# dalab/matrix-manifolds

Hardware: NVIDIA B200
Metric: spd4_pair_dist_grad_evals_per_sec (higher is better)
Workload: dtype f32

## Files before the change

matrix-manifolds_b200/csrc/gm_pairs_spd.cu:

```cuda
#include "gm_product.cuh"

#ifndef GM_N
#error "compile with -DGM_N=<matrix size>"
#endif

namespace gm {

template <class Op, typename T, int KMODE>
__global__ void __launch_bounds__(128)
spd_pair_kernel(Op op, PairSpec ps, const T* __restrict__ xa, const T* __restrict__ xb,
                const T* __restrict__ gout, T coef, T* __restrict__ ga, T* __restrict__ gb,
                T* __restrict__ out_d2, TargetSpec tg, LossCfg lc, T scale_sp, double* __restrict__ acc) {
  constexpr int E = Op::E;
  __shared__ double red[2][4];
  long long k = (long long)blockIdx.x * blockDim.x + threadIdx.x;
  bool active = k < ps.P;
  long long ra = -1, rb = -1;
  double loss_v = 0.0, gd2_v = 0.0;
  T gx[E], gy[E];
  if (active) {
    decode_pair(ps, k, ra, rb);
    T x[E], y[E];
    load_row<T, E>(xa, ra, x);
    load_row<T, E>(xb, rb, y);
    if constexpr (KMODE == K_FWD) {
      out_d2[k] = op.dist2(x, y);
    } else {
      T d2 = op.dist2_grad(x, y, gx, gy);
      T w;
      if constexpr (KMODE == K_BWD) {
        w = coef * gout[k];
      } else {
        T g = fetch_target_ps<T>(ps, tg, k, ra, rb);
        T m = scale_sp * d2;
        T dm;
        T lv = loss_term<T>(lc, g, m, dm);
        loss_v = (double)lv;
        gd2_v = (double)dm * (double)d2;
        w = dm * scale_sp;
        if (out_d2) out_d2[k] = d2;
      }
      GM_UNROLL for (int e = 0; e < E; ++e) { gx[e] *= w; gy[e] *= w; }
    }
  }
  if constexpr (KMODE != K_FWD) {
    if (ps.mode == GM_PAIRS_ELEMENTWISE) {
      if (active) {
        store_row<T, E>(ga, ra, gx);
        store_row<T, E>(gb, rb, gy);
      }
    } else {
      warp_accumulate_row<T, E>(ga, ra, gx);
      warp_accumulate_row<T, E>(gb, rb, gy);
    }
  }
  if constexpr (KMODE == K_FUSED) {
    block_accumulate(loss_v, acc, red[0]);
    block_accumulate(gd2_v, acc + 1, red[1]);
  }
}

template <int BYTES>
__device__ __forceinline__ void cp_async(void* smem, const void* gmem) {
  unsigned s = (unsigned)__cvta_generic_to_shared(smem);
  if constexpr (BYTES == 16)
    asm volatile("cp.async.cg.shared.global [%0], [%1], 16;\n" ::"r"(s), "l"(gmem) : "memory");
  else if constexpr (BYTES == 8)
    asm volatile("cp.async.ca.shared.global [%0], [%1], 8;\n" ::"r"(s), "l"(gmem) : "memory");
  else
    asm volatile("cp.async.ca.shared.global [%0], [%1], 4;\n" ::"r"(s), "l"(gmem) : "memory");
}
__device__ __forceinline__ void cp_async_commit() { asm volatile("cp.async.commit_group;\n" ::: "memory"); }
__device__ __forceinline__ void cp_async_wait_all() { asm volatile("cp.async.wait_group 0;\n" ::: "memory"); }
template <int PENDING>
__device__ __forceinline__ void cp_async_wait_group() { asm volatile("cp.async.wait_group %0;\n" ::"n"(PENDING) : "memory"); }

template <typename T, int E, int STAGES = 2>
struct RowStage {
  static constexpr int ROWB = E * (int)sizeof(T);
  static constexpr int CPB = (ROWB % 16 == 0) ? 16 : ((ROWB % 8 == 0) ? 8 : 4);
  static constexpr int NCH = ROWB / CPB;
  static constexpr int THREADS = 128;
  static constexpr int BYTES = STAGES * 2  * ROWB * THREADS;
  __device__ __forceinline__ static char* slot(char* base, int s, int r, int c, int t) {
    return base + ((((s * 2 + r) * NCH + c) * THREADS + t) * CPB);
  }
  __device__ __forceinline__ static void issue(char* base, int s, int r, int t, const T* row) {
    const char* g = reinterpret_cast<const char*>(row);
    GM_UNROLL for (int c = 0; c < NCH; ++c) cp_async<CPB>(slot(base, s, r, c, t), g + c * CPB);
  }
  __device__ __forceinline__ static void read(char* base, int s, int r, int t, T (&out)[E]) {
    GM_UNROLL for (int c = 0; c < NCH; ++c) {
      if constexpr (CPB == 16) {
        float4 v = *reinterpret_cast<const float4*>(slot(base, s, r, c, t));
        const T* tv = reinterpret_cast<const T*>(&v);
        GM_UNROLL for (int j = 0; j < 16 / (int)sizeof(T); ++j) out[c * (16 / (int)sizeof(T)) + j] = tv[j];
      } else if constexpr (CPB == 8) {
        float2 v = *reinterpret_cast<const float2*>(slot(base, s, r, c, t));
        const T* tv = reinterpret_cast<const T*>(&v);
        GM_UNROLL for (int j = 0; j < 8 / (int)sizeof(T); ++j) out[c * (8 / (int)sizeof(T)) + j] = tv[j];
      } else {
        out[c] = *reinterpret_cast<const T*>(slot(base, s, r, c, t));
      }
    }
  }
};

struct PairCursor {
  long long a, pos;
  int slot;
  __device__ __forceinline__ void init(const PairSpec& ps, long long k0) {
    if (ps.mode == GM_PAIRS_TRIU && k0 < ps.P) {
      long long b;
      triu_decode(k0 + ps.k0, ps.B, a, b);
      pos = b - a - 1;
    } else {
      a = -1; pos = 0; slot = 0;
    }
  }
  __device__ __forceinline__ void rows(const PairSpec& ps, long long k, long long& ra, long long& rb) const {
    if (ps.mode == GM_PAIRS_LIST) {
      ra = load_index(ps.idx_i, k, ps.idx64);
      rb = load_index(ps.idx_j, k, ps.idx64);
    } else if (ps.mode == GM_PAIRS_SAMPLED) {
      const unsigned char* hp;
      rb = (long long)sampled_j(ps, k, ra, hp);
    } else {
      long long b = a + 1 + pos;
      if (ps.nodes) { ra = load_index(ps.nodes, a, ps.idx64); rb = load_index(ps.nodes, b, ps.idx64); }
      else { ra = a; rb = b; }
    }
  }
  __device__ __forceinline__ void rows_sampled(const PairSpec& ps, long long k, long long& ra, long long& rb,
                                               unsigned& hop) {
    const int g = (int)(ps.per_shift >= 0 ? (k >> ps.per_shift) : (k / ps.per_src));
    if (g != a) {
      a = g;
      pos = ((const int*)ps.idx_i)[g];
      slot = ps.slots ? ps.slots[g] : g;
    }
    const unsigned i = (unsigned)pos;
    unsigned j = __umulhi(sample_hash32(ps.seed, (unsigned long long)k), (unsigned)(ps.n_nodes - 1));
    j += (j >= i) ? 1u : 0u;
    hop = load_hop(ps.levels + (long long)slot * ps.n_nodes + j);
    ra = (long long)i;
    rb = (long long)j;
  }
  __device__ __forceinline__ void advance(const PairSpec& ps) {
    if (ps.mode == GM_PAIRS_TRIU) {
      pos += 32;
      while (a < ps.B - 1 && pos >= ps.B - a - 1) { pos -= ps.B - a - 1; ++a; }
    }
  }
};

template <int ROWBYTES, bool SMALL = (ROWBYTES >= 64)> struct RowId { using type = long long; };
template <int ROWBYTES> struct RowId<ROWBYTES, true> { using type = unsigned; };

template <typename T> struct RawScalar;
template <> struct RawScalar<float> {
  using type = unsigned;
  __device__ __forceinline__ static unsigned pack(float v) { return __float_as_uint(v); }
  __device__ __forceinline__ static float unpack(unsigned r) { return __uint_as_float(r); }
};
template <> struct RawScalar<double> {
  using type = unsigned long long;
  __device__ __forceinline__ static unsigned long long pack(double v) { return (unsigned long long)__double_as_longlong(v); }
  __device__ __forceinline__ static double unpack(unsigned long long r) { return __longlong_as_double((long long)r); }
};

template <class Op, typename T, int KMODE, int MINB, int DEPTH, int SPEC = 0>
__global__ void __launch_bounds__(128, MINB)
spd_pair_stream_kernel(Op op, PairSpec ps, const T* __restrict__ xa, const T* __restrict__ xb,
                       const T* __restrict__ gout, T coef, T* __restrict__ ga, T* __restrict__ gb,
                       T* __restrict__ out_d2, TargetSpec tg, LossCfg lc, T scale_sp, double* __restrict__ acc,
                       long long chunk, const ShardTab sh) {
  constexpr int E = Op::E;
  constexpr int N = GM_N;
  constexpr int EU = N * (N + 1) / 2;
  constexpr int D = DEPTH;
  using Stage = RowStage<T, E, D + 1>;
  using Raw = RawScalar<T>;
  using raw_t = typename Raw::type;
  extern __shared__ __align__(16) char stage_mem[];
  __shared__ double red[2][4];
  __shared__ T hop_lut[256];
  const int tid = threadIdx.x, lane = tid & 31;
  const unsigned full = 0xffffffffu;
  const long long warp_id = (long long)blockIdx.x * 4 + (tid >> 5);
  const long long wbase = warp_id * chunk + lane;
  const int nseg = ps.nseg;
  auto locate = [&](int t, long long& k) -> bool {
    int s = 0, o = t;
    if (nseg > 1) {
      s = t / (int)chunk;
      o = t - s * (int)chunk;
      if (s >= nseg) return false;
    } else if (t >= chunk) {
      return false;
    }
    const long long in_seg = wbase + o;
    k = (long long)s * ps.seg_len + in_seg;
    return in_seg < ps.seg_len && k < ps.P;
  };
  [[maybe_unused]] auto locate_so = [&](int s, int o, long long& k) -> bool {
    if (s >= nseg) return false;
    const long long in_seg = wbase + o;
    k = (long long)s * ps.seg_len + in_seg;
    return in_seg < ps.seg_len && k < ps.P;
  };
  const bool hopsP = SPEC ? true : (KMODE == K_FUSED) && tg.mode == GM_TGT_HOPS_PACKED;
  const bool hops8 = SPEC ? true : (KMODE == K_FUSED) && (tg.mode == GM_TGT_HOPS_U8 || hopsP);
  const bool hops16 = SPEC ? false : (KMODE == K_FUSED) && tg.mode == GM_TGT_HOPS_U16;
  const bool rawj = SPEC ? true : hopsP || ps.mode == GM_PAIRS_SAMPLED;
  if (hops8) {
    for (int h = tid; h < 256; h += 128) hop_lut[h] = ((T)h * (T)h) / (T)tg.max_sq;
    __syncthreads();
  }

  using row_t = typename RowId<E * (int)sizeof(T)>::type;
  const row_t kNoRow = (row_t)-1;
  const bool sharded = SPEC ? false : sh.log2w >= 0;
  auto xrow = [&](const T* base, row_t r) -> const T* {
    if (sharded) return (const T*)sh.x[(unsigned)r & sh.mask] + (size_t)((unsigned long long)r >> sh.log2w) * E;
    return base + (size_t)r * E;
  };
  auto grow = [&](T* base, row_t r, long long& lr) -> T* {
    lr = (long long)r;
    if (sharded) { base = (T*)sh.g[(unsigned)r & sh.mask]; lr = (long long)((unsigned long long)r >> sh.log2w); }
    return base;
  };
  int tc = 0;
  PairCursor ahead;
  row_t ra[D + 2], rb[D + 2];
  raw_t tgq[D + 1];
  bool v[D + 2];
  unsigned hopn = 0;
  GM_UNROLL for (int q = 0; q < D + 2; ++q) { ra[q] = kNoRow; rb[q] = kNoRow; v[q] = false; }
  GM_UNROLL for (int q = 0; q < D + 1; ++q) tgq[q] = 0;
  const bool sampled = SPEC ? false : ps.mode == GM_PAIRS_SAMPLED;
  int stage = 0;

  auto fetch_scalar = [&](long long k, row_t ra, row_t rb) -> raw_t {
    if constexpr (KMODE == K_BWD) {
      return Raw::pack(gout[k]);
    } else {
      if (hopsP) return (raw_t)(((unsigned)rb) >> 24);
      if (hops8) return (raw_t)((const unsigned char*)tg.data)[k];
      if (hops16) return (raw_t)((const unsigned short*)tg.data)[k];
      return Raw::pack(fetch_target<T>(tg, k, (long long)ra, (long long)rb));
    }
  };
  auto scalar_value = [&](raw_t r) -> T {
    if constexpr (KMODE == K_BWD) {
      return Raw::unpack(r);
    } else {
      if (hops8) return hop_lut[r];
      if (hops16) { T h = (T)r; return (h * h) / (T)tg.max_sq; }
      return Raw::unpack(r);
    }
  };
  auto load_rows = [&](long long k, row_t& ra, row_t& rb, unsigned& hop) {
    if constexpr (SPEC != 0) {
      ra = (row_t)((const int*)ps.idx_i)[k];
      rb = (row_t)(unsigned)((const int*)ps.idx_j)[k];
      return;
    }
    long long a, b;
    if (sampled) ahead.rows_sampled(ps, k, a, b, hop);
    else ahead.rows(ps, k, a, b);
    ra = (row_t)a; rb = (row_t)b;
  };

  ahead.init(ps, wbase);
  GM_UNROLL for (int q = 0; q < D; ++q) {
    long long kq = 0;
    v[q] = locate(32 * q, kq);
    if (v[q]) {
      unsigned hop = 0;
      load_rows(kq, ra[q], rb[q], hop);
      tgq[q] = (sampled && hopsP) ? (raw_t)hop : fetch_scalar(kq, ra[q], rb[q]);
      if (rawj) rb[q] &= (row_t)0x00ffffffu;
      Stage::issue(stage_mem, q, 0, tid, xrow(xa, ra[q]));
      Stage::issue(stage_mem, q, 1, tid, xrow(xb, rb[q]));
    }
    cp_async_commit();
    ahead.advance(ps);
  }
  {
    long long kq = 0;
    v[D] = locate(32 * D, kq);
    if (v[D]) load_rows(kq, ra[D], rb[D], hopn);
  }
  [[maybe_unused]] int hs = SPEC ? (32 * (D + 1)) / (int)chunk : 0;
  [[maybe_unused]] int ho = SPEC ? 32 * (D + 1) - hs * (int)chunk : 0;

  double loss_v = 0.0, gd2_v = 0.0;
  row_t acc_row = kNoRow;
  T gacc[EU];
  GM_UNROLL for (int e = 0; e < EU; ++e) gacc[e] = (T)0;
  row_t prep_row = kNoRow;
  T ap[Op::kPrepSize];

  auto flush = [&]() {
    if (acc_row != kNoRow) {
      GM_UNROLL for (int e = 0; e < EU; ++e) gacc[e] = warp_sum(gacc[e]);
      if (lane == 0) {
        T gfull[E];
        GM_UNROLL for (int i = 0; i < N; ++i)
          GM_UNROLL for (int j = i; j < N; ++j) {
            gfull[i * N + j] = gacc[i * N - i * (i - 1) / 2 + (j - i)];
            gfull[j * N + i] = gfull[i * N + j];
          }
        long long lr;
        T* gbase = grow(ga, acc_row, lr);
        atomic_add_row<T, E>(gbase, lr, gfull);
      }
      GM_UNROLL for (int e = 0; e < EU; ++e) gacc[e] = (T)0;
      acc_row = kNoRow;
    }
  };

  const int t_end = (nseg > 1 && wbase - lane < ps.seg_len) ? nseg * (int)chunk : 0;
  while (nseg > 1 ? tc < t_end : __any_sync(full, v[0])) {
    cp_async_wait_group<D - 1>();
    const bool v0 = v[0];
    const row_t ra0 = ra[0], rb0 = rb[0];
    const raw_t tg0 = tgq[0];
    T x[E], y[E];
    if (v0) {
      Stage::read(stage_mem, stage, 1, tid, y);
      if (!Op::kCanPrep || ra0 != prep_row) Stage::read(stage_mem, stage, 0, tid, x);
    }
    tgq[D] = 0;
    if (v[D]) {
      long long kq = 0;
      if (KMODE == K_BWD || !hopsP) locate(tc + 32 * D, kq);
      tgq[D] = (sampled && hopsP) ? (raw_t)hopn : fetch_scalar(kq, ra[D], rb[D]);
      if (rawj) rb[D] &= (row_t)0x00ffffffu;
      int sn = stage + D;
      if (sn > D) sn -= D + 1;
      Stage::issue(stage_mem, sn, 0, tid, xrow(xa, ra[D]));
      Stage::issue(stage_mem, sn, 1, tid, xrow(xb, rb[D]));
    }
    cp_async_commit();
    ahead.advance(ps);
    long long kh = 0;
    if constexpr (SPEC != 0) {
      v[D + 1] = locate_so(hs, ho, kh);
      ho += 32;
      if (ho >= (int)chunk) { ho -= (int)chunk; ++hs; }
    } else {
      v[D + 1] = locate(tc + 32 * (D + 1), kh);
    }
    ra[D + 1] = kNoRow; rb[D + 1] = kNoRow;
    unsigned hop_next = 0;
    if (v[D + 1]) load_rows(kh, ra[D + 1], rb[D + 1], hop_next);

    T gx[E], gy[E];
    if (v0) {
      T d2, w;
      [[maybe_unused]] typename Op::EigState st;
      if constexpr (Op::kCanPrep) {
        if (ra0 != prep_row) { op.prep(x, ap); prep_row = ra0; }
        d2 = op.eig_forward_prepped(ap, y, st);
      } else {
        d2 = op.dist2_grad(x, y, gx, gy);
      }
      if constexpr (KMODE == K_BWD) {
        w = coef * scalar_value(tg0);
      } else {
        T m = scale_sp * d2;
        T dm;
        T lv = loss_term<T, true>(lc, scalar_value(tg0), m, dm);
        loss_v += (double)lv;
        gd2_v += (double)dm * (double)d2;
        w = dm * scale_sp;
        if (out_d2) {
          long long k0 = 0;
          locate(tc, k0);
          out_d2[k0] = d2;
        }
      }
      if constexpr (Op::kCanPrep) {
        op.eig_backward(st, w, gx, gy);
      } else {
        GM_UNROLL for (int e = 0; e < E; ++e) { gx[e] *= w; gy[e] *= w; }
      }
      long long lrb;
      T* gbb = grow(gb, rb0, lrb);
      atomic_add_row<T, E>(gbb, lrb, gy);
    }
    {
      row_t r0 = __shfl_sync(full, ra0, 0);
      bool uniform = __all_sync(full, v0 && ra0 == r0);
      if (uniform && r0 == acc_row) {
        GM_UNROLL for (int i = 0; i < N; ++i)
          GM_UNROLL for (int j = i; j < N; ++j) gacc[i * N - i * (i - 1) / 2 + (j - i)] += gx[i * N + j];
      } else {
        flush();
        if (uniform) {
          acc_row = r0;
          GM_UNROLL for (int i = 0; i < N; ++i)
            GM_UNROLL for (int j = i; j < N; ++j) gacc[i * N - i * (i - 1) / 2 + (j - i)] = gx[i * N + j];
        } else if (v0) {
          long long lra;
          T* gba = grow(ga, ra0, lra);
          atomic_add_row<T, E>(gba, lra, gx);
        }
      }
    }
    tc += 32;
    GM_UNROLL for (int q = 0; q < D + 1; ++q) { ra[q] = ra[q + 1]; rb[q] = rb[q + 1]; v[q] = v[q + 1]; }
    GM_UNROLL for (int q = 0; q < D; ++q) tgq[q] = tgq[q + 1];
    hopn = hop_next;
    stage = (stage == D) ? 0 : stage + 1;
  }
  flush();
  if constexpr (KMODE == K_FUSED) {
    block_accumulate(loss_v, acc, red[0]);
    block_accumulate(gd2_v, acc + 1, red[1]);
  }
}

template <class Op, typename T>
static int launch_op(const Op& op, const PairArgs& a) {
  if (a.ps.P <= 0) return 0;
  if (a.px) return a.sh.log2w >= 0 ? GM_EUNSUPPORTED : launch_product<SpdLead<Op>, T>(SpdLead<Op>{op}, a);
  const int threads = 128;
  long long blocks = (a.ps.P + threads - 1) / threads;
  if (blocks > 0x7fffffffLL) return GM_EINVAL;
  dim3 grid((unsigned)blocks), block(threads);
  const T* xa = (const T*)a.xa;
  const T* xb = (const T*)a.xb;
#ifndef GM_MINB_F32
#define GM_MINB_F32 4
#endif
#ifndef GM_PF_DEPTH
#define GM_PF_DEPTH 1
#endif
  constexpr int MINB = sizeof(T) == 4 ? GM_MINB_F32 : 2;
  constexpr int DEPTH = (RowStage<T, Op::E, GM_PF_DEPTH + 1>::BYTES + 3 * 1024) * MINB <= 224 * 1024 ? GM_PF_DEPTH : 1;
  using Stage = RowStage<T, Op::E, DEPTH + 1>;
  if (a.kmode != K_FWD && a.ps.mode != GM_PAIRS_ELEMENTWISE && RowStage<T, Op::E, 2>::BYTES <= 64 * 1024) {
    int dev = 0, sms = 0, occ = 0;
    cudaGetDevice(&dev);
    cudaDeviceGetAttribute(&sms, cudaDevAttrMultiProcessorCount, dev);
    auto launch_stream = [&](auto kern, auto spec_kern, const T* gout, T coef, T* out_d2, T scale, double* acc) -> int {
      cudaFuncSetAttribute(kern, cudaFuncAttributeMaxDynamicSharedMemorySize, Stage::BYTES);
      cudaOccupancyMaxActiveBlocksPerMultiprocessor(&occ, kern, threads, Stage::BYTES);
      if (occ < 1) occ = 1;
      long long max_blocks = (long long)sms * occ;
      long long want = (a.ps.P + threads - 1) / threads;
      long long nb = want < max_blocks ? want : max_blocks;
      long long warps = nb * (threads / 32);
      PairSpec ps = a.ps;
      if (ps.mode != GM_PAIRS_LIST || ps.nseg < 2 || ps.P < ps.nseg * 32LL * warps) ps.nseg = 1;
      ps.seg_len = (ps.P + ps.nseg - 1) / ps.nseg;
      long long chunk = ((ps.seg_len + warps - 1) / warps + 31) / 32 * 32;
      if (chunk * ps.nseg > 0x7fffffffLL) return GM_EINVAL;
#ifndef GM_NO_SPEC
      if constexpr (GM_N == 4 && sizeof(T) == 4 && Op::kCanPrep) {
        if (spec_kern && ps.nseg > 1 && !ps.idx64 && a.tg.mode == GM_TGT_HOPS_PACKED && a.sh.log2w < 0) {
          cudaFuncSetAttribute(spec_kern, cudaFuncAttributeMaxDynamicSharedMemorySize, Stage::BYTES);
          spec_kern<<<(unsigned)nb, threads, Stage::BYTES, a.stream>>>(op, ps, xa, xb, gout, coef, (T*)a.ga, (T*)a.gb,
                                                                    out_d2, a.tg, a.lc, scale, acc, chunk, a.sh);
          note_launch();
          return check_launch();
        }
      }
#endif
      kern<<<(unsigned)nb, threads, Stage::BYTES, a.stream>>>(op, ps, xa, xb, gout, coef, (T*)a.ga, (T*)a.gb, out_d2,
                                                             a.tg, a.lc, scale, acc, chunk, a.sh);
      note_launch();
      return check_launch();
    };
    using kern_t = decltype(&spd_pair_stream_kernel<Op, T, K_FUSED, MINB, DEPTH>);
    if (a.kmode == K_BWD)
      return launch_stream(spd_pair_stream_kernel<Op, T, K_BWD, MINB, DEPTH>, (kern_t) nullptr, (const T*)a.gout,
                           (T)a.coef, nullptr, (T)0, nullptr);
    kern_t spec = nullptr;
    if constexpr (GM_N == 4 && sizeof(T) == 4 && Op::kCanPrep) spec = spd_pair_stream_kernel<Op, T, K_FUSED, MINB, DEPTH, 1>;
    return launch_stream(spd_pair_stream_kernel<Op, T, K_FUSED, MINB, DEPTH>, spec, nullptr, (T)0, (T*)a.out_d2,
                         (T)a.scale_sp, a.acc);
  }
  if (a.sh.log2w >= 0) return GM_EUNSUPPORTED;
  switch (a.kmode) {
    case K_FWD:
      spd_pair_kernel<Op, T, K_FWD><<<grid, block, 0, a.stream>>>(
          op, a.ps, xa, xb, nullptr, (T)0, nullptr, nullptr, (T*)a.out_d2, a.tg, a.lc, (T)0, nullptr);
      break;
    case K_BWD:
      spd_pair_kernel<Op, T, K_BWD><<<grid, block, 0, a.stream>>>(
          op, a.ps, xa, xb, (const T*)a.gout, (T)a.coef, (T*)a.ga, (T*)a.gb, nullptr, a.tg, a.lc, (T)0, nullptr);
      break;
    default:
      spd_pair_kernel<Op, T, K_FUSED><<<grid, block, 0, a.stream>>>(
          op, a.ps, xa, xb, nullptr, (T)0, (T*)a.ga, (T*)a.gb, (T*)a.out_d2, a.tg, a.lc, (T)a.scale_sp, a.acc);
  }
  note_launch();
  return check_launch();
}

template <typename T>
static int launch_typed(const PairArgs& a) {
  constexpr int N = GM_N;
  const bool fe = (a.flags & GM_FAST_EIG) != 0;
  const bool fc = (a.flags & GM_FAST_CHOL) != 0;
  if (a.kind == GM_SPD_AI) {
    if constexpr (N == 2) {
      if (fe && fc) { SpdAI<T, 2, true, true> op{(T)a.wmin, (T)a.wmax}; return launch_op<decltype(op), T>(op, a); }
      if (fe && !fc) { SpdAI<T, 2, true, false> op{(T)a.wmin, (T)a.wmax}; return launch_op<decltype(op), T>(op, a); }
      if (!fe && fc) { SpdAI<T, 2, false, true> op{(T)a.wmin, (T)a.wmax}; return launch_op<decltype(op), T>(op, a); }
    }
    if constexpr (N == 3) {
      if (fe) { SpdAI<T, 3, true, false> op{(T)a.wmin, (T)a.wmax}; return launch_op<decltype(op), T>(op, a); }
    }
    SpdAI<T, N, false, false> op{(T)a.wmin, (T)a.wmax};
    return launch_op<decltype(op), T>(op, a);
  }
  if (a.kind == GM_SPD_STEIN) {
    if constexpr (N == 2) {
      if (fc) { SpdStein<T, 2, true> op{(T)a.wmin, (T)a.wmax}; return launch_op<decltype(op), T>(op, a); }
    }
    SpdStein<T, N, false> op{(T)a.wmin, (T)a.wmax};
    return launch_op<decltype(op), T>(op, a);
  }
  return GM_EINVAL;
}

#define GM_CAT2(a, b) a##b
#define GM_CAT(a, b) GM_CAT2(a, b)
int GM_CAT(spd_launch_, GM_N)(const PairArgs& a) {
  if (a.dtype == GM_F32) return launch_typed<float>(a);
  if (a.dtype == GM_F64) return launch_typed<double>(a);
  return GM_EINVAL;
}

}
```

Before: 15.34 billion.

## Skip staging A rows in specialized SPD kernel; precompute run votes and segment cursor

In the specialized hops-packed kernel, only the B row is staged through cp.async shared memory. The A row is loaded directly from global memory only when the prep row changes, which halves the dynamic shared memory per block. The warp-uniform run vote is moved to issue time and carried in a small queue. The per-iteration segment locate is replaced by an incremental cursor. The A-row load becomes a synchronous global load on the critical path when runs change, and the change adds register pressure.

```diff
diff --git a/matrix-manifolds_b200/csrc/gm_pairs_spd.cu b/matrix-manifolds_b200/csrc/gm_pairs_spd.cu
--- a/matrix-manifolds_b200/csrc/gm_pairs_spd.cu
+++ b/matrix-manifolds_b200/csrc/gm_pairs_spd.cu
@@ -75,15 +75,15 @@
 template <int PENDING>
 __device__ __forceinline__ void cp_async_wait_group() { asm volatile("cp.async.wait_group %0;\n" ::"n"(PENDING) : "memory"); }
 
-template <typename T, int E, int STAGES = 2>
+template <typename T, int E, int STAGES = 2, int ROWS = 2>
 struct RowStage {
   static constexpr int ROWB = E * (int)sizeof(T);
   static constexpr int CPB = (ROWB % 16 == 0) ? 16 : ((ROWB % 8 == 0) ? 8 : 4);
   static constexpr int NCH = ROWB / CPB;
   static constexpr int THREADS = 128;
-  static constexpr int BYTES = STAGES * 2  * ROWB * THREADS;
+  static constexpr int BYTES = STAGES * ROWS * ROWB * THREADS;
   __device__ __forceinline__ static char* slot(char* base, int s, int r, int c, int t) {
-    return base + ((((s * 2 + r) * NCH + c) * THREADS + t) * CPB);
+    return base + ((((s * ROWS + r) * NCH + c) * THREADS + t) * CPB);
   }
   __device__ __forceinline__ static void issue(char* base, int s, int r, int t, const T* row) {
     const char* g = reinterpret_cast<const char*>(row);
@@ -179,7 +179,9 @@
   constexpr int N = GM_N;
   constexpr int EU = N * (N + 1) / 2;
   constexpr int D = DEPTH;
-  using Stage = RowStage<T, E, D + 1>;
+  constexpr bool STAGE_A = SPEC == 0;
+  constexpr int RB = STAGE_A ? 1 : 0;
+  using Stage = RowStage<T, E, D + 1, STAGE_A ? 2 : 1>;
   using Raw = RawScalar<T>;
   using raw_t = typename Raw::type;
   extern __shared__ __align__(16) char stage_mem[];
@@ -203,12 +205,6 @@
     k = (long long)s * ps.seg_len + in_seg;
     return in_seg < ps.seg_len && k < ps.P;
   };
-  [[maybe_unused]] auto locate_so = [&](int s, int o, long long& k) -> bool {
-    if (s >= nseg) return false;
-    const long long in_seg = wbase + o;
-    k = (long long)s * ps.seg_len + in_seg;
-    return in_seg < ps.seg_len && k < ps.P;
-  };
   const bool hopsP = SPEC ? true : (KMODE == K_FUSED) && tg.mode == GM_TGT_HOPS_PACKED;
   const bool hops8 = SPEC ? true : (KMODE == K_FUSED) && (tg.mode == GM_TGT_HOPS_U8 || hopsP);
   const bool hops16 = SPEC ? false : (KMODE == K_FUSED) && tg.mode == GM_TGT_HOPS_U16;
@@ -235,8 +231,15 @@
   row_t ra[D + 2], rb[D + 2];
   raw_t tgq[D + 1];
   bool v[D + 2];
+  constexpr bool RUNQ = SPEC != 0;
+  bool uq[D + 1];
   unsigned hopn = 0;
   GM_UNROLL for (int q = 0; q < D + 2; ++q) { ra[q] = kNoRow; rb[q] = kNoRow; v[q] = false; }
+  GM_UNROLL for (int q = 0; q < D + 1; ++q) uq[q] = false;
+  auto vote_run = [&](int q) {
+    const row_t r0 = __shfl_sync(full, ra[q], 0);
+    uq[q] = __all_sync(full, v[q] && ra[q] == r0);
+  };
   GM_UNROLL for (int q = 0; q < D + 1; ++q) tgq[q] = 0;
   const bool sampled = SPEC ? false : ps.mode == GM_PAIRS_SAMPLED;
   int stage = 0;
@@ -272,7 +275,7 @@
     ra = (row_t)a; rb = (row_t)b;
   };
 
-  ahead.init(ps, wbase);
+  if constexpr (SPEC == 0) ahead.init(ps, wbase);
   GM_UNROLL for (int q = 0; q < D; ++q) {
     long long kq = 0;
     v[q] = locate(32 * q, kq);
@@ -281,11 +284,12 @@
       load_rows(kq, ra[q], rb[q], hop);
       tgq[q] = (sampled && hopsP) ? (raw_t)hop : fetch_scalar(kq, ra[q], rb[q]);
       if (rawj) rb[q] &= (row_t)0x00ffffffu;
-      Stage::issue(stage_mem, q, 0, tid, xrow(xa, ra[q]));
-      Stage::issue(stage_mem, q, 1, tid, xrow(xb, rb[q]));
-    }
+      if (STAGE_A) Stage::issue(stage_mem, q, 0, tid, xrow(xa, ra[q]));
+      Stage::issue(stage_mem, q, RB, tid, xrow(xb, rb[q]));
+    }
+    if constexpr (RUNQ) vote_run(q);
     cp_async_commit();
-    ahead.advance(ps);
+    if constexpr (SPEC == 0) ahead.advance(ps);
   }
   {
     long long kq = 0;
@@ -294,6 +298,14 @@
   }
   [[maybe_unused]] int hs = SPEC ? (32 * (D + 1)) / (int)chunk : 0;
   [[maybe_unused]] int ho = SPEC ? 32 * (D + 1) - hs * (int)chunk : 0;
+  [[maybe_unused]] long long hk = 0, hend = 0;
+  [[maybe_unused]] auto enter_segment = [&]() {
+    const long long sb = (long long)hs * ps.seg_len;
+    hk = sb + wbase + ho;
+    const long long e = sb + ps.seg_len < ps.P ? sb + ps.seg_len : ps.P;
+    hend = hs < nseg ? e : 0;
+  };
+  if constexpr (SPEC != 0) enter_segment();
 
   double loss_v = 0.0, gd2_v = 0.0;
   row_t acc_row = kNoRow;
@@ -329,9 +341,10 @@
     const raw_t tg0 = tgq[0];
     T x[E], y[E];
     if (v0) {
-      Stage::read(stage_mem, stage, 1, tid, y);
-      if (!Op::kCanPrep || ra0 != prep_row) Stage::read(stage_mem, stage, 0, tid, x);
-    }
+      Stage::read(stage_mem, stage, RB, tid, y);
+      if (STAGE_A && (!Op::kCanPrep || ra0 != prep_row)) Stage::read(stage_mem, stage, 0, tid, x);
+    }
+    if constexpr (RUNQ) vote_run(D);
     tgq[D] = 0;
     if (v[D]) {
       long long kq = 0;
@@ -340,17 +353,19 @@
       if (rawj) rb[D] &= (row_t)0x00ffffffu;
       int sn = stage + D;
       if (sn > D) sn -= D + 1;
-      Stage::issue(stage_mem, sn, 0, tid, xrow(xa, ra[D]));
-      Stage::issue(stage_mem, sn, 1, tid, xrow(xb, rb[D]));
+      if (STAGE_A) Stage::issue(stage_mem, sn, 0, tid, xrow(xa, ra[D]));
+      Stage::issue(stage_mem, sn, RB, tid, xrow(xb, rb[D]));
     }
     cp_async_commit();
-    ahead.advance(ps);
     long long kh = 0;
     if constexpr (SPEC != 0) {
-      v[D + 1] = locate_so(hs, ho, kh);
+      v[D + 1] = hk < hend;
+      kh = hk;
+      hk += 32;
       ho += 32;
-      if (ho >= (int)chunk) { ho -= (int)chunk; ++hs; }
-    } else {
+      if (ho >= (int)chunk) { ho -= (int)chunk; ++hs; enter_segment(); }
+    } else {
+      ahead.advance(ps);
       v[D + 1] = locate(tc + 32 * (D + 1), kh);
     }
     ra[D + 1] = kNoRow; rb[D + 1] = kNoRow;
@@ -362,7 +377,11 @@
       T d2, w;
       [[maybe_unused]] typename Op::EigState st;
       if constexpr (Op::kCanPrep) {
-        if (ra0 != prep_row) { op.prep(x, ap); prep_row = ra0; }
+        if (ra0 != prep_row) {
+          if (!STAGE_A) load_row<T, E>(xa, (long long)ra0, x);
+          op.prep(x, ap);
+          prep_row = ra0;
+        }
         d2 = op.eig_forward_prepped(ap, y, st);
       } else {
         d2 = op.dist2_grad(x, y, gx, gy);
@@ -392,8 +411,14 @@
       atomic_add_row<T, E>(gbb, lrb, gy);
     }
     {
-      row_t r0 = __shfl_sync(full, ra0, 0);
-      bool uniform = __all_sync(full, v0 && ra0 == r0);
+      row_t r0 = ra0;
+      bool uniform;
+      if constexpr (RUNQ) {
+        uniform = uq[0];
+      } else {
+        r0 = __shfl_sync(full, ra0, 0);
+        uniform = __all_sync(full, v0 && ra0 == r0);
+      }
       if (uniform && r0 == acc_row) {
         GM_UNROLL for (int i = 0; i < N; ++i)
           GM_UNROLL for (int j = i; j < N; ++j) gacc[i * N - i * (i - 1) / 2 + (j - i)] += gx[i * N + j];
@@ -412,7 +437,7 @@
     }
     tc += 32;
     GM_UNROLL for (int q = 0; q < D + 1; ++q) { ra[q] = ra[q + 1]; rb[q] = rb[q + 1]; v[q] = v[q + 1]; }
-    GM_UNROLL for (int q = 0; q < D; ++q) tgq[q] = tgq[q + 1];
+    GM_UNROLL for (int q = 0; q < D; ++q) { tgq[q] = tgq[q + 1]; uq[q] = uq[q + 1]; }
     hopn = hop_next;
     stage = (stage == D) ? 0 : stage + 1;
   }
@@ -442,6 +467,7 @@
   constexpr int MINB = sizeof(T) == 4 ? GM_MINB_F32 : 2;
   constexpr int DEPTH = (RowStage<T, Op::E, GM_PF_DEPTH + 1>::BYTES + 3 * 1024) * MINB <= 224 * 1024 ? GM_PF_DEPTH : 1;
   using Stage = RowStage<T, Op::E, DEPTH + 1>;
+  using SpecStage = RowStage<T, Op::E, DEPTH + 1, 1>;
   if (a.kmode != K_FWD && a.ps.mode != GM_PAIRS_ELEMENTWISE && RowStage<T, Op::E, 2>::BYTES <= 64 * 1024) {
     int dev = 0, sms = 0, occ = 0;
     cudaGetDevice(&dev);
@@ -462,8 +488,8 @@
 #ifndef GM_NO_SPEC
       if constexpr (GM_N == 4 && sizeof(T) == 4 && Op::kCanPrep) {
         if (spec_kern && ps.nseg > 1 && !ps.idx64 && a.tg.mode == GM_TGT_HOPS_PACKED && a.sh.log2w < 0) {
-          cudaFuncSetAttribute(spec_kern, cudaFuncAttributeMaxDynamicSharedMemorySize, Stage::BYTES);
-          spec_kern<<<(unsigned)nb, threads, Stage::BYTES, a.stream>>>(op, ps, xa, xb, gout, coef, (T*)a.ga, (T*)a.gb,
+          cudaFuncSetAttribute(spec_kern, cudaFuncAttributeMaxDynamicSharedMemorySize, SpecStage::BYTES);
+          spec_kern<<<(unsigned)nb, threads, SpecStage::BYTES, a.stream>>>(op, ps, xa, xb, gout, coef, (T*)a.ga, (T*)a.gb,
                                                                     out_d2, a.tg, a.lc, scale, acc, chunk, a.sh);
           note_launch();
           return check_launch();
```

Result: faster. 15.81 billion, median of 6 (+3.1%).
